# VatsalSy/gerris-fft-particles

Hardware: AMD Instinct MI355X
Metric: Mcell-steps/s (projection+advection), 3D 256^3 uniform (higher is better)
Workload: dtype f64; 1 GPU; 3-D periodic Taylor-Green, 256^3 per GPU, default projection/advection parameters (SURVEY 8d config C); relax_mode=exact, parallelism=1 box, rccl_world_size=0

## Files before the change

gerris-fft-particles_amd/csrc/timestep_kernels.hip:

```cpp
#include "gfship_internal.hpp"
#include "cell_loop.hpp"
#include <cfloat>

namespace gfship {

#define EXT_PROLOGUE(L)							\
  int i = blockIdx.x*blockDim.x + threadIdx.x;				\
  int j = blockIdx.y;							\
  int k = (L).dim == 3 ? blockIdx.z : 0;				\
  if (i > (L).n) return;						\
  long c = (L).idx (i, j, k)

static inline void ext_grid (const Layout & L, dim3 * grid, dim3 * block)
{
  int b = L.n >= 256 ? 256 : L.n >= 128 ? 128 : 64;
  *block = dim3 (b);
  *grid = dim3 ((L.n + 1 + b - 1)/b, L.n + 1, L.dim == 3 ? L.n + 1 : 1);
}

struct Ptr3  { double * p[3]; };
struct CPtr3 { const double * p[3]; };
struct Ptr6  { double * p[6]; };
struct CPtr6 { const double * p[6]; };
struct Visc3 { double d[3]; double g[3]; };
// ... 1653 lines not shown
};

#define SW_RING 128

template <bool VL, bool SRC>
__device__ __forceinline__ void sweep_ring_path (SweepLds & S_, const Layout & L, const CPtr3 & v, const CPtr3 & un,
						 const CPtr3 & gm, double dt, const Visc3 & src3, int rid)
{
  const int n = L.n;
  const double rn = (double) n, rsize2 = (double) n/2.;
  const int sy = (int) L.sy, sz = (int) L.sz;
  const int kb = blockIdx.z*SWZ;
  auto plane = [n, sz] (int k) { return (k < 1 ? k + n : k > n ? k - n : k)*sz; };
  int role = -1, hd = 0, hcol = 0, hslot = 0;
  if (rid < 2*SWX) {
    role = rid < SWX ? 0 : 1; hd = 1; hslot = rid % SWX;
    int hj = blockIdx.y*SWY + (role ? SWY + 1 : 0);
    hj = hj < 1 ? hj + n : hj > n ? hj - n : hj;
    hcol = (int) L.idx (blockIdx.x*SWX + hslot + 1, hj, 0);
  }
  else if (rid < 2*SWX + 2*SWY) {
    role = rid < 2*SWX + SWY ? 2 : 3; hd = 0; hslot = (rid - 2*SWX) % SWY;
    int hi_ = blockIdx.x*SWX + (role == 3 ? SWX + 1 : 0);
    hi_ = hi_ < 1 ? hi_ + n : hi_ > n ? hi_ - n : hi_;
    hcol = (int) L.idx (hi_, blockIdx.y*SWY + hslot + 1, 0);
  }
  const bool ring = role >= 0, ring_minus = role == 0 || role == 2;
  const int hoff = hd == 0 ? 1 : sy;
  const int ry = role == 0 ? 0 : role == 1 ? SWY + 1 : hslot + 1;
  const int rx = role == 2 ? 0 : role == 3 ? SWX + 1 : hslot + 1;
  double hvm[3], hv0[3] = { 0., 0., 0. }, hvp[3] = { 0., 0., 0. }, hvn[3] = { 0., 0., 0. };
  double hunb = 0., hunzb = 0., hlo[3] = { 0., 0., 0. }, hgmo[3] = { 0., 0., 0. };
  if (ring) {
#pragma unroll
    for (int q = 0; q < 3; q++) {
      hv0[q] = v.p[q][hcol + plane (kb - 1)];
      hvp[q] = v.p[q][hcol + plane (kb)];
      hvn[q] = v.p[q][hcol + plane (kb + 1)];
    }
    hunzb = un.p[2][hcol + plane (kb - 1)];
  }
  for (int p = kb; p <= kb + SWZ + 1; p++) {
    const int zp = plane (p);
    Stencil7 HW[3];
    double hua[3] = { 0., 0., 0. }, hub[3] = { 0., 0., 0. };
#pragma unroll
    for (int q = 0; q < 3; q++) {
      hvm[q] = hv0[q]; hv0[q] = hvp[q]; hvp[q] = hvn[q];
      HW[q].v0 = hv0[q];
      HW[q].m[0] = HW[q].p[0] = HW[q].m[1] = HW[q].p[1] = 0.;
      HW[q].m[2] = hvm[q]; HW[q].p[2] = hvp[q];
    }
    if (ring) {
      const int hc = hcol + zp;
#pragma unroll
      for (int q = 0; q < 3; q++) {
	hvn[q] = v.p[q][hcol + plane (p + 2)];
	HW[q].m[0] = v.p[q][hc - 1];  HW[q].p[0] = v.p[q][hc + 1];
	HW[q].m[1] = v.p[q][hc - sy]; HW[q].p[1] = v.p[q][hc + sy];
      }
      hua[0] = un.p[0][hc]; hub[0] = un.p[0][hc - 1];
      hua[1] = un.p[1][hc]; hub[1] = un.p[1][hc - sy];
      hua[2] = un.p[2][hc]; hub[2] = hunzb;
#pragma unroll
      for (int q = 0; q < 3; q++)
	S_.V[q][ry][rx] = hv0[q];
      if (role == 2) S_.UNx[hslot][0] = hua[0];
      if (role == 0) S_.UNy[0][hslot] = hua[1];
    }
    __syncthreads ();
    double hl[3] = { 0., 0., 0. }, hr[3] = { 0., 0., 0. };
    if (ring) {
      const AdvShared S = adv_shared_v (hua, hub, dt, rsize2);
#pragma unroll
      for (int q = 0; q < 3; q++) {
	const FacePair f = hd == 0 ? adv_face_values_s<0, VL, SRC> (HW[q], S, dt, rsize2, src3.g[q]) :
	  adv_face_values_s<1, VL, SRC> (HW[q], S, dt, rsize2, src3.g[q]);
	hl[q] = f.l; hr[q] = f.r;
      }
      if (p > kb && ring_minus) {
	const int ho = hcol + plane (p - 1);
	const double ua = hunb;
	const double fu = 1.*ua*dt*rn;
#pragma unroll
	for (int q = 0; q < 3; q++) {
	  const double rs = role == 2 ? S_.FRx[q][hslot][0] : S_.FRy[q][0][hslot];
	  double f = fu;
	  f *= upwinded (ua, hlo[q], rs) - face_interp (hgmo[q], gm.p[q][ho + hoff])*dt/2.;
	  if (role == 2) S_.FPx[q][hslot][0] = f; else S_.FPy[q][0][hslot] = f;
	}
      }
    }
    __syncthreads ();
    if (ring) {
#pragma unroll
      for (int q = 0; q < 3; q++) {
	if (role == 3) S_.FRx[q][hslot][SWX] = hr[q];
	if (role == 1) S_.FRy[q][SWY][hslot] = hr[q];
	hlo[q] = hl[q];
	hgmo[q] = gm.p[q][hcol + zp];
      }
      hunb = hua[hd];
      hunzb = hua[2];
    }
  }
}

template <bool VL, bool SRC, bool CORR>
__global__ void __launch_bounds__(SWN + SW_RING)
advect3_sweep_kernel (Layout L, CPtr3 v, Ptr3 out, CPtr3 un, CPtr3 gm, CPtr3 gc, double dt, Visc3 src3,
		      AdvCorr K)
{
  __shared__ SweepLds S_;
  const int tid = threadIdx.x;
  if (tid >= SWN) {
    sweep_ring_path<VL, SRC> (S_, L, v, un, gm, dt, src3, tid - SWN);
    return;
  }
  const int tx = tid % SWX, ty = tid / SWX;
  const int n = L.n;
  const double rn = (double) n, rsize2 = (double) n/2.;
  const int sy = (int) L.sy, sz = (int) L.sz;
  const int i = blockIdx.x*SWX + tx + 1, j = blockIdx.y*SWY + ty + 1;
  const int kb = blockIdx.z*SWZ;
  const int col = (int) L.idx (i, j, 0);
  auto plane = [n, sz] (int k) { return (k < 1 ? k + n : k > n ? k - n : k)*sz; };

  double vm[3], v0[3], vp[3], vn[3];
  double una[3], unb[3];
  double flo[3][3];
  double fpz[3] = { 0., 0., 0. };
  double gmo[3];
  double low[3] = { 0., 0., 0. };
#pragma unroll
  for (int q = 0; q < 3; q++) {
    v0[q] = v.p[q][col + plane (kb - 1)];
    vp[q] = v.p[q][col + plane (kb)];
    vn[q] = v.p[q][col + plane (kb + 1)];
    gmo[q] = gm.p[q][col + plane (kb)];
#pragma unroll
    for (int d = 0; d < 3; d++) flo[q][d] = 0.;
  }
#pragma unroll
  for (int d = 0; d < 3; d++) {
    una[d] = un.p[d][col + plane (kb - 1)];
    unb[d] = 0.;
  }

  for (int p = kb; p <= kb + SWZ + 1; p++) {
    const int zp = plane (p);
#pragma unroll
    for (int q = 0; q < 3; q++) {
      vm[q] = v0[q]; v0[q] = vp[q]; vp[q] = vn[q];
      vn[q] = v.p[q][col + plane (p + 2)];
    }
    const double unzb = una[2];
#pragma unroll
    for (int d = 0; d < 3; d++) {
      unb[d] = una[d];
      una[d] = un.p[d][col + zp];
    }
#pragma unroll
    for (int q = 0; q < 3; q++)
      S_.V[q][ty + 1][tx + 1] = v0[q];
    S_.UNx[ty][tx + 1] = una[0];
    S_.UNy[ty + 1][tx] = una[1];
    __syncthreads ();
    SweepFv F[3];
    {
      const double b[3] = { S_.UNx[ty][tx], S_.UNy[ty][tx], unzb };
      const AdvShared S = adv_shared_v (una, b, dt, rsize2);
#pragma unroll
      for (int q = 0; q < 3; q++) {
	Stencil7 W;
	W.v0 = v0[q];
	W.m[0] = S_.V[q][ty + 1][tx];     W.p[0] = S_.V[q][ty + 1][tx + 2];
	W.m[1] = S_.V[q][ty][tx + 1];     W.p[1] = S_.V[q][ty + 2][tx + 1];
	W.m[2] = vm[q];                   W.p[2] = vp[q];
	F[q] = sweep_face_values<VL, SRC> (W, S, dt, rsize2, src3.g[q]);
      }
    }
    double Fp[3][3];
    if (p > kb) {
      const int co = col + plane (p - 1);
      const double fux = 1.*unb[0]*dt*rn, fuy = 1.*unb[1]*dt*rn, fuz = 1.*unb[2]*dt*rn;
#pragma unroll
      for (int q = 0; q < 3; q++) {
	const double g0 = gmo[q];
	const double gx = gm.p[q][co + 1], gy = gm.p[q][co + sy], gz = gm.p[q][col + zp];
	double f = fux;
	f *= upwinded (unb[0], flo[q][0], S_.FRx[q][ty][tx + 1]) - face_interp (g0, gx)*dt/2.;
	Fp[q][0] = f;
	f = fuy;
	f *= upwinded (unb[1], flo[q][1], S_.FRy[q][ty + 1][tx]) - face_interp (g0, gy)*dt/2.;
	Fp[q][1] = f;
	f = fuz;
	f *= upwinded (unb[2], flo[q][2], F[q].r[2]) - face_interp (g0, gz)*dt/2.;
	Fp[q][2] = f;
	gmo[q] = gz;
	S_.FPx[q][ty][tx + 1] = Fp[q][0];
	S_.FPy[q][ty + 1][tx] = Fp[q][1];
      }
    }
    __syncthreads ();
    if (p > kb) {
      const int o = p - 1, co = col + plane (o);
      if (p > kb + 1) {
	const int k = o;
	const unsigned J = n - j, K_ = n - k;
	const bool back_first = __ffs (~J) > __ffs (~K_);
	double res[3];
#pragma unroll
	for (int q = 0; q < 3; q++) {
	  const double Fmx = S_.FPx[q][ty][tx], Fmy = S_.FPy[q][ty][tx], Fmz = fpz[q];
	  double acc = 0.;
	  if (i > 1)
	    acc += Fmx;
	  acc -= Fp[q][0];
	  acc -= Fp[q][1];
	  acc -= Fp[q][2];
	  if (back_first) {
	    if (k > 1) acc += Fmz;
	    if (j > 1) acc += Fmy;
	  }
	  else {
	    if (j > 1) acc += Fmy;
	    if (k > 1) acc += Fmz;
	  }
	  if (i == 1)
	    acc += Fmx;
	  if (j == 1)
	    acc += Fmy;
	  if (k == 1)
	    acc += Fmz;
	  double val = vm[q];
	  val += acc/1.;
	  const double gcv = gc.p[q] ? gc.p[q][co] : 0.;
	  if (gc.p[q])
	    val -= gcv*dt;
	  if (SRC && src3.g[q] != 0.) {
	    double sum = 0;
	    sum += src3.g[q];
	    val += dt*sum;
	  }
	  if (CORR)
	    val = val - gcv*K.dt;
	  out.p[q][co] = val;
	  res[q] = val;
	}
	if (CORR && K.uc[0]) {
	  if (k & 1) {
#pragma unroll
	    for (int q = 0; q < 3; q++) low[q] = res[q];
	  }
	  else {
	    const int lane = tid & 63, lx = lane & 31;
	    const bool head = !(lane & 32) && !(lx & 1);
	    const int src[4] = { lx + 32, lx + 33, lx, lx + 1 };
#pragma unroll
	    for (int q = 0; q < 3; q++) {
	      double val = 0., sa = 0.;
#pragma unroll
	      for (int id = 0; id < 4; id++) { val += __shfl (res[q], src[id], 64)*1.; sa += 1.; }
#pragma unroll
	      for (int id = 0; id < 4; id++) { val += __shfl (low[q], src[id], 64)*1.; sa += 1.; }
	      if (head)
		K.uc[q][K.Lc.idx ((i + 1)/2, (j + 1)/2, k/2)] = val/sa;
	    }
	  }
	}
      }
#pragma unroll
      for (int q = 0; q < 3; q++)
	fpz[q] = Fp[q][2];
    }
#pragma unroll
    for (int q = 0; q < 3; q++) {
#pragma unroll
      for (int d = 0; d < 3; d++)
	flo[q][d] = F[q].l[d];
      S_.FRx[q][ty][tx] = F[q].r[0];
      S_.FRy[q][ty][tx] = F[q].r[1];
    }
  }
}

struct Sweep2Lds {
  double V[3][SWY + 2][SWX + 2];
  double UNx[SWY][SWX + 1], UNy[SWY + 1][SWX];
  double FRx[2][3][SWY][SWX + 1], FRy[2][3][SWY + 1][SWX];
  double FPx[3][SWY][SWX + 1], FPy[3][SWY + 1][SWX];
  double GM[3][SWY + 1][SWX + 1];
  double FL[3][3][SWY][SWX];
};

template <bool MPI>
__device__ __forceinline__ int sweep2_plane (int k, int n, int sz, bool zlo, bool zhi)
{
  if (k < 1) k = MPI && zlo ? (k < 0 ? 0 : k) : k + n;
  else if (k > n) k = MPI && zhi ? n + 1 : k - n;
  return k*sz;
}

template <bool VL, bool SRC, bool MPI>
__device__ __forceinline__ void sweep2_ring_path (Sweep2Lds & S_, const Layout & L, const CPtr3 & v, const CPtr3 & un,
						  const CPtr3 & gm, double dt, const Visc3 & src3, int rid,
						  const GhostFv & G)
{
  const int n = L.n;
  const double rn = (double) n, rsize2 = (double) n/2.;
  const int sy0 = (int) L.sy, sz = (int) L.sz;
  const int kb = blockIdx.z*SWZ;
  const bool zlo = MPI && G.r[5] != nullptr, zhi = MPI && G.r[4] != nullptr;
  auto plane = [=] (int k) { return sweep2_plane<MPI> (k, n, sz, zlo, zhi); };
  int role = -1, hd = 0, hcol = 0, hslot = 0;
  const double * recv = nullptr;
  if (rid < 2*SWX) {
    role = rid < SWX ? 0 : 1; hd = 1; hslot = rid % SWX;
    int hj = blockIdx.y*SWY + (role ? SWY + 1 : 0);
    if (MPI && (hj < 1 || hj > n) && G.r[role ? 2 : 3])
      recv = G.r[role ? 2 : 3] + (blockIdx.x*SWX + hslot);
    else
      hj = hj < 1 ? hj + n : hj > n ? hj - n : hj;
    hcol = (int) L.idx (blockIdx.x*SWX + hslot + 1, hj, 0);
  }
  else if (rid < 2*SWX + 2*SWY) {
    role = rid < 2*SWX + SWY ? 2 : 3; hd = 0; hslot = (rid - 2*SWX) % SWY;
    int hi_ = blockIdx.x*SWX + (role == 3 ? SWX + 1 : 0);
    if (MPI && (hi_ < 1 || hi_ > n) && G.r[role == 3 ? 0 : 1])
      recv = G.r[role == 3 ? 0 : 1] + (blockIdx.y*SWY + hslot);
    else
      hi_ = hi_ < 1 ? hi_ + n : hi_ > n ? hi_ - n : hi_;
    hcol = (int) L.idx (hi_, blockIdx.y*SWY + hslot + 1, 0);
  }
  const int sy = MPI && recv && hd == 1 ? 0 : sy0;
  const size_t nf = (size_t) n*n;
  const bool ring = role >= 0, ring_minus = role == 0 || role == 2;
  const int hoff = MPI && recv && !ring_minus ? 0 : hd == 0 ? 1 : sy0;
  const int ry = role == 0 ? 0 : role == 1 ? SWY + 1 : hslot + 1;
  const int rx = role == 2 ? 0 : role == 3 ? SWX + 1 : hslot + 1;
  double hvm[3], hv0[3] = { 0., 0., 0. }, hvp[3] = { 0., 0., 0. }, hvn[3] = { 0., 0., 0. };
  double nbn[3][4];
  double huan[3] = { 0., 0., 0. }, hubn[2] = { 0., 0. };
  double hunb = 0., hunzb = 0., hlo[3] = { 0., 0., 0. }, hgmo[3], hgmn[3] = { 0., 0., 0. };
  double hgcn[3] = { 0., 0., 0. };
#pragma unroll
  for (int q = 0; q < 3; q++) {
    hgmo[q] = 0.;
#pragma unroll
    for (int e = 0; e < 4; e++) nbn[q][e] = 0.;
  }
  if (ring) {
    const int hc = hcol + plane (kb);
#pragma unroll
    for (int q = 0; q < 3; q++) {
      hv0[q] = v.p[q][hcol + plane (kb - 1)];
      hvp[q] = v.p[q][hc];
      hvn[q] = v.p[q][hcol + plane (kb + 1)];
      nbn[q][0] = v.p[q][hc - 1];  nbn[q][1] = v.p[q][hc + 1];
      nbn[q][2] = v.p[q][hc - sy]; nbn[q][3] = v.p[q][hc + sy];
    }
    huan[0] = un.p[0][hc]; hubn[0] = un.p[0][hc - 1];
    huan[1] = un.p[1][hc]; hubn[1] = un.p[1][hc - sy];
    huan[2] = un.p[2][hc];
    hunzb = un.p[2][hcol + plane (kb - 1)];
  }
  for (int p = kb; p <= kb + SWZ + 1; p++) {
    const int zp = plane (p);
    Stencil7 HW[3];
    double hua[3], hub[3];
#pragma unroll
    for (int q = 0; q < 3; q++) {
      hvm[q] = hv0[q]; hv0[q] = hvp[q]; hvp[q] = hvn[q];
      HW[q].v0 = hv0[q];
      HW[q].m[0] = nbn[q][0]; HW[q].p[0] = nbn[q][1];
      HW[q].m[1] = nbn[q][2]; HW[q].p[1] = nbn[q][3];
      HW[q].m[2] = hvm[q]; HW[q].p[2] = hvp[q];
      hgmo[q] = hgmn[q];
    }
    hua[0] = huan[0]; hua[1] = huan[1]; hua[2] = huan[2];
    hub[0] = hubn[0]; hub[1] = hubn[1]; hub[2] = hunzb;
    const double hgc[3] = { hgcn[0], hgcn[1], hgcn[2] };
    if (ring) {
      const int hc1 = hcol + plane (p + 1);
#pragma unroll
      for (int q = 0; q < 3; q++) {
	hvn[q] = v.p[q][hcol + plane (p + 2)];
	nbn[q][0] = v.p[q][hc1 - 1];  nbn[q][1] = v.p[q][hc1 + 1];
	nbn[q][2] = v.p[q][hc1 - sy]; nbn[q][3] = v.p[q][hc1 + sy];
	hgmn[q] = gm.p[q][hcol + zp];
	hgcn[q] = gm.p[q][hcol + zp + hoff];
      }
      huan[0] = un.p[0][hc1]; hubn[0] = un.p[0][hc1 - 1];
      huan[1] = un.p[1][hc1]; hubn[1] = un.p[1][hc1 - sy];
      huan[2] = un.p[2][hc1];
#pragma unroll
      for (int q = 0; q < 3; q++) {
	S_.V[q][ry][rx] = hv0[q];
	if (role == 3) S_.GM[q][hslot][SWX] = hgmo[q];
	if (role == 1) S_.GM[q][SWY][hslot] = hgmo[q];
      }
      if (role == 2) S_.UNx[hslot][0] = hua[0];
      if (role == 0) S_.UNy[0][hslot] = hua[1];
    }
    __syncthreads ();
    double hl[3] = { 0., 0., 0. };
    if (ring) {
      const AdvShared S = adv_shared_v (hua, hub, dt, rsize2);
#pragma unroll
      for (int q = 0; q < 3; q++) {
	FacePair f = hd == 0 ? adv_face_values_s<0, VL, SRC> (HW[q], S, dt, rsize2, src3.g[q]) :
	  adv_face_values_s<1, VL, SRC> (HW[q], S, dt, rsize2, src3.g[q]);
	if (MPI && recv) {
	  const int zc = p < 1 ? 0 : p > n ? n - 1 : p - 1;
	  f.l = f.r = recv[q*nf + (size_t) n*zc];
	}
	hl[q] = f.l;
	if (role == 3) S_.FRx[p & 1][q][hslot][SWX] = f.r;
	if (role == 1) S_.FRy[p & 1][q][SWY][hslot] = f.r;
      }
      if (p > kb && ring_minus) {
	const double ua = hunb;
	const double fu = 1.*ua*dt*rn;
#pragma unroll
	for (int q = 0; q < 3; q++) {
	  const double rs = role == 2 ? S_.FRx[(p - 1) & 1][q][hslot][0] : S_.FRy[(p - 1) & 1][q][0][hslot];
	  double f = fu;
	  f *= upwinded (ua, hlo[q], rs) - face_interp (hgmo[q], hgc[q])*dt/2.;
	  if (role == 2) S_.FPx[q][hslot][0] = f; else S_.FPy[q][0][hslot] = f;
	}
      }
    }
    __syncthreads ();
    if (ring) {
#pragma unroll
      for (int q = 0; q < 3; q++)
	hlo[q] = hl[q];
      hunb = hua[hd];
      hunzb = hua[2];
    }
  }
}

template <bool VL, bool SRC, bool CORR, bool MPI>
__global__ void __launch_bounds__(SWN + SW_RING)
advect3_sweep2_kernel (Layout L, CPtr3 v, Ptr3 out, CPtr3 un, CPtr3 gm, CPtr3 gc, double dt, Visc3 src3,
		       AdvCorr K, GhostFv G)
{
  __shared__ Sweep2Lds S_;
  const int tid = threadIdx.x;
  if (tid >= SWN) {
    sweep2_ring_path<VL, SRC, MPI> (S_, L, v, un, gm, dt, src3, tid - SWN, G);
    return;
  }
  const int tx = tid % SWX, ty = tid / SWX;
  const int n = L.n;
  const double rn = (double) n, rsize2 = (double) n/2.;
  const int sz = (int) L.sz;
  const int i = blockIdx.x*SWX + tx + 1, j = blockIdx.y*SWY + ty + 1;
  const int kb = blockIdx.z*SWZ;
  const int col = (int) L.idx (i, j, 0);
  const bool zlo = MPI && G.r[5] != nullptr, zhi = MPI && G.r[4] != nullptr;
  auto plane = [=] (int k) { return sweep2_plane<MPI> (k, n, sz, zlo, zhi); };
  const size_t nf = (size_t) n*n;
  const int fpos = (i - 1) + n*(j - 1);

  double vm[3], v0[3], vp[3], vn[3];
  double una[3], unb[3], unn[3];
  double fpz[3] = { 0., 0., 0. };
  double gmo[3], gmc[3];
  double low[3] = { 0., 0., 0. };
#pragma unroll
  for (int q = 0; q < 3; q++) {
    v0[q] = v.p[q][col + plane (kb - 1)];
    vp[q] = v.p[q][col + plane (kb)];
    vn[q] = v.p[q][col + plane (kb + 1)];
    gmo[q] = 0.;
    gmc[q] = gm.p[q][col + plane (kb - 1)];
#pragma unroll
    for (int d = 0; d < 3; d++) S_.FL[q][d][ty][tx] = 0.;
  }
#pragma unroll
  for (int d = 0; d < 3; d++) {
    una[d] = un.p[d][col + plane (kb - 1)];
    unn[d] = un.p[d][col + plane (kb)];
    unb[d] = 0.;
  }

  for (int p = kb; p <= kb + SWZ + 1; p++) {
    const int zp = plane (p);
    const int rp = p & 1, ro = rp ^ 1;
    double gcv[3];
#pragma unroll
    for (int q = 0; q < 3; q++) {
      vm[q] = v0[q]; v0[q] = vp[q]; vp[q] = vn[q];
      vn[q] = v.p[q][col + plane (p + 2)];
      gmo[q] = gmc[q];
      gmc[q] = gm.p[q][col + zp];
      gcv[q] = gc.p[q] ? gc.p[q][col + plane (p - 1)] : 0.;
    }
    const double unzb = una[2];
#pragma unroll
    for (int d = 0; d < 3; d++) {
      unb[d] = una[d];
      una[d] = unn[d];
      unn[d] = un.p[d][col + plane (p + 1)];
    }
#pragma unroll
    for (int q = 0; q < 3; q++) {
      S_.V[q][ty + 1][tx + 1] = v0[q];
      S_.GM[q][ty][tx] = gmo[q];
    }
    S_.UNx[ty][tx + 1] = una[0];
    S_.UNy[ty + 1][tx] = una[1];
    __syncthreads ();
    double flz[3] = { 0., 0., 0. };
    if (p > kb) {
      const double fux = 1.*unb[0]*dt*rn, fuy = 1.*unb[1]*dt*rn;
#pragma unroll
      for (int q = 0; q < 3; q++) {
	const double g0 = gmo[q];
	double f = fux;
	f *= upwinded (unb[0], S_.FL[q][0][ty][tx], S_.FRx[ro][q][ty][tx + 1]) - face_interp (g0, S_.GM[q][ty][tx + 1])*dt/2.;
	S_.FPx[q][ty][tx + 1] = f;
	f = fuy;
	f *= upwinded (unb[1], S_.FL[q][1][ty][tx], S_.FRy[ro][q][ty + 1][tx]) - face_interp (g0, S_.GM[q][ty + 1][tx])*dt/2.;
	S_.FPy[q][ty + 1][tx] = f;
	flz[q] = S_.FL[q][2][ty][tx];
      }
    }
    double frz[3];
    {
      const double b[3] = { S_.UNx[ty][tx], S_.UNy[ty][tx], unzb };
      const AdvShared S = adv_shared_v (una, b, dt, rsize2);
#pragma unroll
      for (int q = 0; q < 3; q++) {
	Stencil7 W;
	W.v0 = v0[q];
	W.m[0] = S_.V[q][ty + 1][tx];     W.p[0] = S_.V[q][ty + 1][tx + 2];
	W.m[1] = S_.V[q][ty][tx + 1];     W.p[1] = S_.V[q][ty + 2][tx + 1];
	W.m[2] = vm[q];                   W.p[2] = vp[q];
	const SweepFv F = sweep_face_values<VL, SRC> (W, S, dt, rsize2, src3.g[q]);
	S_.FRx[rp][q][ty][tx] = F.r[0];
	S_.FRy[rp][q][ty][tx] = F.r[1];
	frz[q] = F.r[2];
#pragma unroll
	for (int d = 0; d < 3; d++)
	  S_.FL[q][d][ty][tx] = F.l[d];
	if (MPI) {
	  if (zlo && p == 0) S_.FL[q][2][ty][tx] = G.r[5][q*nf + fpos];
	  if (zhi && p == n + 1) frz[q] = G.r[4][q*nf + fpos];
	}
      }
    }
    double Fpz[3] = { 0., 0., 0. };
    if (p > kb) {
      const double fuz = 1.*unb[2]*dt*rn;
#pragma unroll
      for (int q = 0; q < 3; q++) {
	double f = fuz;
	f *= upwinded (unb[2], flz[q], frz[q]) - face_interp (gmo[q], gmc[q])*dt/2.;
	Fpz[q] = f;
      }
    }
    __syncthreads ();
    if (p > kb) {
      const int o = p - 1, co = col + plane (o);
      if (p > kb + 1) {
	const int k = o;
	const unsigned J = n - j, K_ = n - k;
	const bool back_first = __ffs (~J) > __ffs (~K_);
	double res[3];
#pragma unroll
	for (int q = 0; q < 3; q++) {
	  const double Fmx = S_.FPx[q][ty][tx], Fmy = S_.FPy[q][ty][tx], Fmz = fpz[q];
	  const double Fpx = S_.FPx[q][ty][tx + 1], Fpy = S_.FPy[q][ty + 1][tx];
	  double acc = 0.;
	  if (i > 1)
	    acc += Fmx;
	  acc -= Fpx;
	  acc -= Fpy;
	  acc -= Fpz[q];
	  if (back_first) {
	    if (k > 1) acc += Fmz;
	    if (j > 1) acc += Fmy;
	  }
	  else {
	    if (j > 1) acc += Fmy;
	    if (k > 1) acc += Fmz;
	  }
	  if (i == 1)
	    acc += Fmx;
	  if (j == 1)
	    acc += Fmy;
	  if (k == 1)
	    acc += Fmz;
	  double val = vm[q];
	  val += acc/1.;
	  if (gc.p[q])
	    val -= gcv[q]*dt;
	  if (SRC && src3.g[q] != 0.) {
	    double sum = 0;
	    sum += src3.g[q];
	    val += dt*sum;
	  }
	  if (CORR)
	    val = val - gcv[q]*K.dt;
	  out.p[q][co] = val;
	  res[q] = val;
	}
	if (CORR && K.uc[0]) {
	  if (k & 1) {
#pragma unroll
	    for (int q = 0; q < 3; q++) low[q] = res[q];
	  }
	  else {
	    const int lane = tid & 63, lx = lane & 31;
	    const bool head = !(lane & 32) && !(lx & 1);
	    const int src[4] = { lx + 32, lx + 33, lx, lx + 1 };
#pragma unroll
	    for (int q = 0; q < 3; q++) {
	      double val = 0., sa = 0.;
#pragma unroll
	      for (int id = 0; id < 4; id++) { val += __shfl (res[q], src[id], 64)*1.; sa += 1.; }
#pragma unroll
	      for (int id = 0; id < 4; id++) { val += __shfl (low[q], src[id], 64)*1.; sa += 1.; }
	      if (head)
		K.uc[q][K.Lc.idx ((i + 1)/2, (j + 1)/2, k/2)] = val/sa;
	    }
	  }
	}
      }
#pragma unroll
      for (int q = 0; q < 3; q++)
	fpz[q] = Fpz[q];
    }
  }
}

struct PredLds {
  double V[3][SWY + 2][SWX + 2];
  double FRx[2][SWY][SWX + 1], FRy[2][SWY + 1][SWX];
  double UOx[SWY][SWX + 1], UOy[SWY + 1][SWX];
};

template <int D, bool VL, bool VS>
__device__ __forceinline__ FacePair cen_face_values_s (const Stencil7 & W, const double uc[3], double dt,
						       int n, double visc, double gsrc)
{
  const double rsize = (double) n, rsize2 = (double) n/2.;
  constexpr int A = D == 0 ? 1 : 0, B = D == 2 ? 1 : 2;
  const double ta = adv_transverse_v (W.m[A], W.p[A], W.v0, uc[A], dt, rsize2);
  const double tb = adv_transverse_v (W.m[B], W.p[B], W.v0, uc[B], dt, rsize2);
  const double unorm = dt*uc[D]*rsize;
  const double v0 = W.v0, v1 = W.m[D], v2 = W.p[D];
  const double g = VL ? van_leer_gradient (v0, v1, v2) : center_gradient (v0, v1, v2);
  const double vl = v0 + GMIN ((1. - unorm)/2., 0.5)*g;
  const double vr = v0 + GMAX ((- 1. - unorm)/2., -0.5)*g;
  double msrc = 0.;
  if (VS && visc != 0.) {
    const double rh2 = (double) n*(double) n;
    double ga = 0., gb = 0.;
#pragma unroll
    for (int cc = 0; cc < 3; cc++) {
      ga += visc*1.; gb += visc*W.p[cc];
      ga += visc*1.; gb += visc*W.m[cc];
    }
    msrc = 0. + 1.*(gb - ga*v0)*rh2;
  }
  if (VS) msrc += gsrc;
  const double src = dt*msrc/2.;
  double dv = ta;
  dv += tb;
  FacePair f;
  f.l = vl + src - dv;
  f.r = vr + src - dv;
  return f;
}

template <bool VL, bool VS, bool MPI>
__device__ __forceinline__ void pred_ring_path (PredLds & S_, const Layout & L, const CPtr3 & u, double dt,
						const Visc3 & visc, int rid, const Ptr3 & un, const GhostFv & G)
{
  const int n = L.n;
  const int sy0 = (int) L.sy, sz = (int) L.sz;
  const int kb = blockIdx.z*SWZ;
  const bool zlo = MPI && G.r[5] != nullptr, zhi = MPI && G.r[4] != nullptr;
  auto plane = [=] (int k) { return sweep2_plane<MPI> (k, n, sz, zlo, zhi); };
  int role = -1, hd = 0, hcol = 0, hslot = 0;
  const double * recv = nullptr;
  if (rid < 2*SWX) {
    role = rid < SWX ? 0 : 1; hd = 1; hslot = rid % SWX;
    int hj = blockIdx.y*SWY + (role ? SWY + 1 : 0);
    if (MPI && (hj < 1 || hj > n) && G.r[role ? 2 : 3])
      recv = G.r[role ? 2 : 3] + (blockIdx.x*SWX + hslot);
    else
      hj = hj < 1 ? hj + n : hj > n ? hj - n : hj;
    hcol = (int) L.idx (blockIdx.x*SWX + hslot + 1, hj, 0);
  }
  else if (rid < 2*SWX + 2*SWY) {
    role = rid < 2*SWX + SWY ? 2 : 3; hd = 0; hslot = (rid - 2*SWX) % SWY;
    int hi_ = blockIdx.x*SWX + (role == 3 ? SWX + 1 : 0);
    if (MPI && (hi_ < 1 || hi_ > n) && G.r[role == 3 ? 0 : 1])
      recv = G.r[role == 3 ? 0 : 1] + (blockIdx.y*SWY + hslot);
    else
      hi_ = hi_ < 1 ? hi_ + n : hi_ > n ? hi_ - n : hi_;
    hcol = (int) L.idx (hi_, blockIdx.y*SWY + hslot + 1, 0);
  }
  const bool ring = role >= 0, ring_minus = role == 0 || role == 2;
  const int sy = MPI && recv && hd == 1 ? 0 : sy0;
  const int hoff = MPI && recv && !ring_minus ? 0 : hd == 0 ? 1 : sy0;
  const int ry = role == 0 ? 0 : role == 1 ? SWY + 1 : hslot + 1;
  const int rx = role == 2 ? 0 : role == 3 ? SWX + 1 : hslot + 1;
  double hvm[3], hv0[3] = { 0., 0., 0. }, hvp[3] = { 0., 0., 0. }, hvn[3] = { 0., 0., 0. };
  double hlo = 0., hnb = 0., hnbn = 0.;
  double nbn[4] = { 0., 0., 0., 0. };
  if (ring) {
#pragma unroll
    for (int q = 0; q < 3; q++) {
      hv0[q] = u.p[q][hcol + plane (kb - 1)];
      hvp[q] = u.p[q][hcol + plane (kb)];
      hvn[q] = u.p[q][hcol + plane (kb + 1)];
    }
    hnbn = u.p[hd][hcol + hoff + plane (kb - 1)];
    const double * __restrict__ const w = u.p[hd];
    const int hc = hcol + plane (kb);
    nbn[0] = w[hc - 1];  nbn[1] = w[hc + 1];
    nbn[2] = w[hc - sy]; nbn[3] = w[hc + sy];
  }
  for (int p = kb; p <= kb + SWZ + 1; p++) {
    const int zp = plane (p);
    Stencil7 HW;
    HW.m[0] = HW.p[0] = HW.m[1] = HW.p[1] = 0.;
#pragma unroll
    for (int q = 0; q < 3; q++) {
      hvm[q] = hv0[q]; hv0[q] = hvp[q]; hvp[q] = hvn[q];
    }
    HW.v0 = hv0[hd]; HW.m[2] = hvm[hd]; HW.p[2] = hvp[hd];
    HW.m[0] = nbn[0]; HW.p[0] = nbn[1]; HW.m[1] = nbn[2]; HW.p[1] = nbn[3];
    hnb = hnbn;
    if (ring) {
      const int hc1 = hcol + plane (p + 1);
#pragma unroll
      for (int q = 0; q < 3; q++)
	hvn[q] = u.p[q][hcol + plane (p + 2)];
      const double * __restrict__ const w = u.p[hd];
      nbn[0] = w[hc1 - 1];  nbn[1] = w[hc1 + 1];
      nbn[2] = w[hc1 - sy]; nbn[3] = w[hc1 + sy];
      hnbn = w[hcol + hoff + zp];
#pragma unroll
      for (int q = 0; q < 3; q++)
	S_.V[q][ry][rx] = hv0[q];
    }
    __syncthreads ();
    double hl = 0., hr = 0.;
    if (ring) {
      const FacePair f = hd == 0 ? cen_face_values_s<0, VL, VS> (HW, hv0, dt, n, visc.d[0], visc.g[0]) :
	cen_face_values_s<1, VL, VS> (HW, hv0, dt, n, visc.d[1], visc.g[1]);
      hl = f.l; hr = f.r;
      if (MPI && recv) {
	const int zc = p < 1 ? 0 : p > n ? n - 1 : p - 1;
	hl = hr = recv[(size_t) n*zc];
      }
      if (role == 3) S_.FRx[p & 1][hslot][SWX] = hr;
      if (role == 1) S_.FRy[p & 1][SWY][hslot] = hr;
      if (p > kb && ring_minus) {
	const double rs = role == 2 ? S_.FRx[(p - 1) & 1][hslot][0] : S_.FRy[(p - 1) & 1][0][hslot];
	const double s0 = face_interp (hvm[hd], hnb);
	const double val = upwinded (s0, hlo, rs);
	if (role == 2) S_.UOx[hslot][0] = val; else S_.UOy[0][hslot] = val;
	if (MPI && recv && p - 1 >= 1 && p - 1 <= n)
	  un.p[hd][hcol + plane (p - 1)] = val;
      }
    }
    __syncthreads ();
    hlo = hl;
  }
}

template <bool VL, bool VS, bool DIV, bool MPI>
__global__ void __launch_bounds__(SWN + SW_RING)
predict_un_sweep_kernel (Layout L, CPtr3 u, Ptr3 un, double dt, Visc3 visc, double * __restrict__ div,
			 double div_dt, GhostFv G)
{
  __shared__ PredLds S_;
  const int tid = threadIdx.x;
  if (tid >= SWN) {
    pred_ring_path<VL, VS, MPI> (S_, L, u, dt, visc, tid - SWN, un, G);
    return;
  }
  const int tx = tid % SWX, ty = tid / SWX;
  const int n = L.n;
  const int sy = (int) L.sy, sz = (int) L.sz;
  const int i = blockIdx.x*SWX + tx + 1, j = blockIdx.y*SWY + ty + 1;
  const int kb = blockIdx.z*SWZ;
  const int col = (int) L.idx (i, j, 0);
  const bool zlo = MPI && G.r[5] != nullptr, zhi = MPI && G.r[4] != nullptr;
  const bool xmpi = MPI && G.r[1] != nullptr, ympi = MPI && G.r[3] != nullptr;
  auto plane = [=] (int k) { return sweep2_plane<MPI> (k, n, sz, zlo, zhi); };
  const int fpos = (i - 1) + n*(j - 1);
  double vm[3], v0[3], vp[3], vn[3];
  double flo[3] = { 0., 0., 0. };
  double uxp = 0., uyp = 0.;
  double unzo = 0.;
#pragma unroll
  for (int q = 0; q < 3; q++) {
    v0[q] = u.p[q][col + plane (kb - 1)];
    vp[q] = u.p[q][col + plane (kb)];
    vn[q] = u.p[q][col + plane (kb + 1)];
  }
  for (int p = kb; p <= kb + SWZ + 1; p++) {
#pragma unroll
    for (int q = 0; q < 3; q++) {
      vm[q] = v0[q]; v0[q] = vp[q]; vp[q] = vn[q];
      vn[q] = u.p[q][col + plane (p + 2)];
      S_.V[q][ty + 1][tx + 1] = v0[q];
    }
    __syncthreads ();
    const int rp = p & 1, ro = rp ^ 1;
    FacePair F[3];
    double uxpn, uypn;
    {
      Stencil7 W;
      W.v0 = v0[0];
      W.m[0] = S_.V[0][ty + 1][tx];  W.p[0] = S_.V[0][ty + 1][tx + 2];
      W.m[1] = S_.V[0][ty][tx + 1];  W.p[1] = S_.V[0][ty + 2][tx + 1];
      W.m[2] = vm[0];                W.p[2] = vp[0];
      uxpn = W.p[0];
      F[0] = cen_face_values_s<0, VL, VS> (W, v0, dt, n, visc.d[0], visc.g[0]);
      S_.FRx[rp][ty][tx] = F[0].r;
      W.v0 = v0[1];
      W.m[0] = S_.V[1][ty + 1][tx];  W.p[0] = S_.V[1][ty + 1][tx + 2];
      W.m[1] = S_.V[1][ty][tx + 1];  W.p[1] = S_.V[1][ty + 2][tx + 1];
      W.m[2] = vm[1];                W.p[2] = vp[1];
      uypn = W.p[1];
      F[1] = cen_face_values_s<1, VL, VS> (W, v0, dt, n, visc.d[1], visc.g[1]);
      S_.FRy[rp][ty][tx] = F[1].r;
      W.v0 = v0[2];
      W.m[0] = S_.V[2][ty + 1][tx];  W.p[0] = S_.V[2][ty + 1][tx + 2];
      W.m[1] = S_.V[2][ty][tx + 1];  W.p[1] = S_.V[2][ty + 2][tx + 1];
      W.m[2] = vm[2];                W.p[2] = vp[2];
      F[2] = cen_face_values_s<2, VL, VS> (W, v0, dt, n, visc.d[2], visc.g[2]);
      if (MPI) {
	if (zlo && p == 0) F[2].l = G.r[5][fpos];
	if (zhi && p == n + 1) F[2].r = G.r[4][fpos];
      }
    }
    double unv[3] = { 0., 0., 0. };
    if (p > kb) {
      const int o = p - 1, co = col + plane (o);
      unv[0] = upwinded (face_interp (vm[0], uxp), flo[0], S_.FRx[ro][ty][tx + 1]);
      unv[1] = upwinded (face_interp (vm[1], uyp), flo[1], S_.FRy[ro][ty + 1][tx]);
      unv[2] = upwinded (face_interp (vm[2], v0[2]), flo[2], F[2].r);
      if (o >= 1 && o <= n) {
	un.p[0][co] = unv[0];
	un.p[1][co] = unv[1];
	un.p[2][co] = unv[2];
	if (i == n && !xmpi) un.p[0][co - n] = unv[0];
	if (j == n && !ympi) un.p[1][co - n*sy] = unv[1];
	if (o == n && !zlo) un.p[2][co - n*sz] = unv[2];
      }
      else if (MPI && zlo && o == 0)
	un.p[2][co] = unv[2];
      if (DIV) {
	S_.UOx[ty][tx + 1] = unv[0];
	S_.UOy[ty + 1][tx] = unv[1];
      }
    }
// ... 668 lines not shown
```

Measured before the change: 2841 Mcell-steps/s.

## Read ring-lane stencil neighbours from LDS and add corner fill lanes

Ring lanes in the advection sweep previously loaded four neighbour velocities per component from global memory each plane. Now each ring lane loads only its single outward neighbour and reads the rest from the shared V tile, while four extra lanes fill the tile corners. The gc face value is also taken from the shared GM tile instead of a separate global load. Empty asm barriers force prefetched loads to complete before the next iteration, and the interior loop reorders its gc and v loads with a branchless gc pointer. The effect depends on whether the ring-lane loads were on the critical path; the asm fences could serialise memory latency.

```diff
diff --git a/gerris-fft-particles_amd/csrc/timestep_kernels.hip b/gerris-fft-particles_amd/csrc/timestep_kernels.hip
--- a/gerris-fft-particles_amd/csrc/timestep_kernels.hip
+++ b/gerris-fft-particles_amd/csrc/timestep_kernels.hip
@@ -1979,6 +1979,11 @@
   return k*sz;
 }
 
+__device__ __forceinline__ void sweep2_landed (double & x)
+{
+  asm volatile ("" : "+v" (x));
+}
+
 template <bool VL, bool SRC, bool MPI>
 __device__ __forceinline__ void sweep2_ring_path (Sweep2Lds & S_, const Layout & L, const CPtr3 & v, const CPtr3 & un,
 						  const CPtr3 & gm, double dt, const Visc3 & src3, int rid,
@@ -2012,30 +2017,46 @@
   }
   const int sy = MPI && recv && hd == 1 ? 0 : sy0;
   const size_t nf = (size_t) n*n;
-  const bool ring = role >= 0, ring_minus = role == 0 || role == 2;
-  const int hoff = MPI && recv && !ring_minus ? 0 : hd == 0 ? 1 : sy0;
-  const int ry = role == 0 ? 0 : role == 1 ? SWY + 1 : hslot + 1;
-  const int rx = role == 2 ? 0 : role == 3 ? SWX + 1 : hslot + 1;
+  const bool ring_minus = role == 0 || role == 2;
+  int ry = role == 0 ? 0 : role == 1 ? SWY + 1 : hslot + 1;
+  int rx = role == 2 ? 0 : role == 3 ? SWX + 1 : hslot + 1;
+  if (role < 0 && rid < 2*SWX + 2*SWY + 4) {
+    const int e = rid - 2*SWX - 2*SWY;
+    role = 4;
+    int hi_ = blockIdx.x*SWX + (e & 1 ? SWX + 1 : 0), hj = blockIdx.y*SWY + (e & 2 ? SWY + 1 : 0);
+    if (!(MPI && (hi_ < 1 || hi_ > n) && G.r[e & 1 ? 0 : 1]))
+      hi_ = hi_ < 1 ? hi_ + n : hi_ > n ? hi_ - n : hi_;
+    if (!(MPI && (hj < 1 || hj > n) && G.r[e & 2 ? 2 : 3]))
+      hj = hj < 1 ? hj + n : hj > n ? hj - n : hj;
+    hcol = (int) L.idx (hi_, hj, 0);
+    ry = e & 2 ? SWY + 1 : 0; rx = e & 1 ? SWX + 1 : 0;
+  }
+  static_assert (2*SWX + 2*SWY + 4 <= SW_RING, "the ring and the four corners are one lane each");
+  const bool ring = role >= 0 && role < 4, fills = role >= 0;
+  const int hout = role == 0 ? -sy : role == 1 ? sy : role == 2 ? -1 : 1;
+  const int li = ry*(SWX + 2) + rx;
+  const int ln[4] = { role == 2 ? li : li - 1, role == 3 ? li : li + 1,
+		      role == 0 ? li : li - (SWX + 2), role == 1 ? li : li + (SWX + 2) };
   double hvm[3], hv0[3] = { 0., 0., 0. }, hvp[3] = { 0., 0., 0. }, hvn[3] = { 0., 0., 0. };
-  double nbn[3][4];
+  double nbo[3] = { 0., 0., 0. };
   double huan[3] = { 0., 0., 0. }, hubn[2] = { 0., 0. };
-  double hunb = 0., hunzb = 0., hlo[3] = { 0., 0., 0. }, hgmo[3], hgmn[3] = { 0., 0., 0. };
-  double hgcn[3] = { 0., 0., 0. };
-#pragma unroll
-  for (int q = 0; q < 3; q++) {
-    hgmo[q] = 0.;
-#pragma unroll
-    for (int e = 0; e < 4; e++) nbn[q][e] = 0.;
+  double hunb = 0., hunzb = 0., hlo[3] = { 0., 0., 0. }, hgmo[3] = { 0., 0., 0. }, hgmn[3] = { 0., 0., 0. };
+  double hrcn[3] = { 0., 0., 0. };
+  auto recv_at = [=] (int q, int k) { return recv[q*nf + (size_t) n*(k < 1 ? 0 : k > n ? n - 1 : k - 1)]; };
+  if (fills) {
+#pragma unroll
+    for (int q = 0; q < 3; q++) {
+      hv0[q] = v.p[q][hcol + plane (kb - 1)];
+      hvp[q] = v.p[q][hcol + plane (kb)];
+      hvn[q] = v.p[q][hcol + plane (kb + 1)];
+    }
   }
   if (ring) {
     const int hc = hcol + plane (kb);
 #pragma unroll
     for (int q = 0; q < 3; q++) {
-      hv0[q] = v.p[q][hcol + plane (kb - 1)];
-      hvp[q] = v.p[q][hc];
-      hvn[q] = v.p[q][hcol + plane (kb + 1)];
-      nbn[q][0] = v.p[q][hc - 1];  nbn[q][1] = v.p[q][hc + 1];
-      nbn[q][2] = v.p[q][hc - sy]; nbn[q][3] = v.p[q][hc + sy];
+      nbo[q] = v.p[q][hc + hout];
+      if (MPI && recv) hrcn[q] = recv_at (q, kb);
     }
     huan[0] = un.p[0][hc]; hubn[0] = un.p[0][hc - 1];
     huan[1] = un.p[1][hc]; hubn[1] = un.p[1][hc - sy];
@@ -2044,36 +2065,36 @@
   }
   for (int p = kb; p <= kb + SWZ + 1; p++) {
     const int zp = plane (p);
-    Stencil7 HW[3];
-    double hua[3], hub[3];
+    double hua[3], hub[3], hno[3], hrc[3];
 #pragma unroll
     for (int q = 0; q < 3; q++) {
       hvm[q] = hv0[q]; hv0[q] = hvp[q]; hvp[q] = hvn[q];
-      HW[q].v0 = hv0[q];
-      HW[q].m[0] = nbn[q][0]; HW[q].p[0] = nbn[q][1];
-      HW[q].m[1] = nbn[q][2]; HW[q].p[1] = nbn[q][3];
-      HW[q].m[2] = hvm[q]; HW[q].p[2] = hvp[q];
+      hno[q] = nbo[q];
+      hrc[q] = hrcn[q];
       hgmo[q] = hgmn[q];
     }
     hua[0] = huan[0]; hua[1] = huan[1]; hua[2] = huan[2];
     hub[0] = hubn[0]; hub[1] = hubn[1]; hub[2] = hunzb;
-    const double hgc[3] = { hgcn[0], hgcn[1], hgcn[2] };
+    if (fills) {
+#pragma unroll
+      for (int q = 0; q < 3; q++) {
+	hvn[q] = v.p[q][hcol + plane (p + 2)];
+	S_.V[q][ry][rx] = hv0[q];
+      }
+    }
     if (ring) {
       const int hc1 = hcol + plane (p + 1);
 #pragma unroll
       for (int q = 0; q < 3; q++) {
-	hvn[q] = v.p[q][hcol + plane (p + 2)];
-	nbn[q][0] = v.p[q][hc1 - 1];  nbn[q][1] = v.p[q][hc1 + 1];
-	nbn[q][2] = v.p[q][hc1 - sy]; nbn[q][3] = v.p[q][hc1 + sy];
+	nbo[q] = v.p[q][hc1 + hout];
 	hgmn[q] = gm.p[q][hcol + zp];
-	hgcn[q] = gm.p[q][hcol + zp + hoff];
+	if (MPI && recv) hrcn[q] = recv_at (q, p + 1);
       }
       huan[0] = un.p[0][hc1]; hubn[0] = un.p[0][hc1 - 1];
       huan[1] = un.p[1][hc1]; hubn[1] = un.p[1][hc1 - sy];
       huan[2] = un.p[2][hc1];
 #pragma unroll
       for (int q = 0; q < 3; q++) {
-	S_.V[q][ry][rx] = hv0[q];
 	if (role == 3) S_.GM[q][hslot][SWX] = hgmo[q];
 	if (role == 1) S_.GM[q][SWY][hslot] = hgmo[q];
       }
@@ -2086,12 +2107,20 @@
       const AdvShared S = adv_shared_v (hua, hub, dt, rsize2);
 #pragma unroll
       for (int q = 0; q < 3; q++) {
-	FacePair f = hd == 0 ? adv_face_values_s<0, VL, SRC> (HW[q], S, dt, rsize2, src3.g[q]) :
-	  adv_face_values_s<1, VL, SRC> (HW[q], S, dt, rsize2, src3.g[q]);
-	if (MPI && recv) {
-	  const int zc = p < 1 ? 0 : p > n ? n - 1 : p - 1;
-	  f.l = f.r = recv[q*nf + (size_t) n*zc];
-	}
+	const double * Vq = &S_.V[q][0][0];
+	Stencil7 HW;
+	HW.v0 = hv0[q];
+	HW.m[0] = Vq[ln[0]]; HW.p[0] = Vq[ln[1]];
+	HW.m[1] = Vq[ln[2]]; HW.p[1] = Vq[ln[3]];
+	if (role == 2) HW.m[0] = hno[q];
+	if (role == 3) HW.p[0] = hno[q];
+	if (role == 0) HW.m[1] = hno[q];
+	if (role == 1) HW.p[1] = hno[q];
+	HW.m[2] = hvm[q]; HW.p[2] = hvp[q];
+	FacePair f = hd == 0 ? adv_face_values_s<0, VL, SRC> (HW, S, dt, rsize2, src3.g[q]) :
+	  adv_face_values_s<1, VL, SRC> (HW, S, dt, rsize2, src3.g[q]);
+	if (MPI && recv)
+	  f.l = f.r = hrc[q];
 	hl[q] = f.l;
 	if (role == 3) S_.FRx[p & 1][q][hslot][SWX] = f.r;
 	if (role == 1) S_.FRy[p & 1][q][SWY][hslot] = f.r;
@@ -2102,8 +2131,9 @@
 #pragma unroll
 	for (int q = 0; q < 3; q++) {
 	  const double rs = role == 2 ? S_.FRx[(p - 1) & 1][q][hslot][0] : S_.FRy[(p - 1) & 1][q][0][hslot];
+	  const double hgc = role == 2 ? S_.GM[q][hslot][0] : S_.GM[q][0][hslot];
 	  double f = fu;
-	  f *= upwinded (ua, hlo[q], rs) - face_interp (hgmo[q], hgc[q])*dt/2.;
+	  f *= upwinded (ua, hlo[q], rs) - face_interp (hgmo[q], hgc)*dt/2.;
 	  if (role == 2) S_.FPx[q][hslot][0] = f; else S_.FPy[q][0][hslot] = f;
 	}
       }
@@ -2116,6 +2146,12 @@
       hunb = hua[hd];
       hunzb = hua[2];
     }
+#pragma unroll
+    for (int q = 0; q < 3; q++) {
+      sweep2_landed (hvn[q]); sweep2_landed (nbo[q]); sweep2_landed (hgmn[q]); sweep2_landed (huan[q]);
+      if (MPI) sweep2_landed (hrcn[q]);
+    }
+    sweep2_landed (hubn[0]); sweep2_landed (hubn[1]);
   }
 }
 
@@ -2163,6 +2199,10 @@
     unn[d] = un.p[d][col + plane (kb)];
     unb[d] = 0.;
   }
+  const double * gcl[3];
+#pragma unroll
+  for (int q = 0; q < 3; q++)
+    gcl[q] = gc.p[q] ? gc.p[q] : gm.p[q];
 
   for (int p = kb; p <= kb + SWZ + 1; p++) {
     const int zp = plane (p);
@@ -2171,11 +2211,15 @@
 #pragma unroll
     for (int q = 0; q < 3; q++) {
       vm[q] = v0[q]; v0[q] = vp[q]; vp[q] = vn[q];
-      vn[q] = v.p[q][col + plane (p + 2)];
       gmo[q] = gmc[q];
       gmc[q] = gm.p[q][col + zp];
-      gcv[q] = gc.p[q] ? gc.p[q][col + plane (p - 1)] : 0.;
-    }
+    }
+#pragma unroll
+    for (int q = 0; q < 3; q++)
+      gcv[q] = gcl[q][col + plane (p - 1)];
+#pragma unroll
+    for (int q = 0; q < 3; q++)
+      vn[q] = v.p[q][col + plane (p + 2)];
     const double unzb = una[2];
 #pragma unroll
     for (int d = 0; d < 3; d++) {
@@ -2241,6 +2285,10 @@
       }
     }
     __syncthreads ();
+#pragma unroll
+    for (int q = 0; q < 3; q++) {
+      sweep2_landed (vn[q]); sweep2_landed (unn[q]);
+    }
     if (p > kb) {
       const int o = p - 1, co = col + plane (o);
       if (p > kb + 1) {
```

Result: faster. 2889 Mcell-steps/s, median of 6 (+1.7%).
